# zhizdev/sparsefusion

Measured on AMD Instinct MI355X. Metric: novel views/sec, distillation steps (2 NGP renders fwd+bwd + VAE enc/dec + 51-eval PLMS + LPIPS), 256^2 / 32x32 latents, 2-view synthetic hydrant, higher is better.
Workload: dtype bf16 MFMA operands / f32 accumulate (UNet); f32 (NGP render)

## Files before the change

include/sparsefusion_hip.h:

```cpp
#ifndef SPARSEFUSION_HIP_H
#define SPARSEFUSION_HIP_H

#include <stdint.h>

#ifdef __cplusplus
extern "C" {
#endif

#define SF_OK 0
#define SF_ERR_INVALID 1
#define SF_ERR_LAUNCH 2

const char* sf_last_error(void);
int sf_abi_version(void);
int sf_operand_is_f16(void);


int sf_grid_encode_forward(const float* inputs, const float* embeddings,
                           const int32_t* offsets, float* outputs,
                           uint32_t B, uint32_t D, uint32_t C, uint32_t L,
                           float S, uint32_t H, float* dy_dx,
                           uint32_t gridtype, int align_corners,
                           const int32_t* h_offsets, void* stream);

// ... 188 lines not shown
  float* exp_avg;
  float* exp_avg_sq;
  uint64_t n;
  float step_size;
  float pad_;
} sf_adam_tensor;
typedef struct {
  sf_adam_tensor t[SF_ADAM_MAX_TENSORS];
  uint32_t chunk_start[SF_ADAM_MAX_TENSORS];
  uint32_t n_tensors;
  float beta1, beta2, eps;
  float bias_correction2_sqrt;
  float one_minus_beta1, one_minus_beta2;
} sf_adam_args;
int sf_adam_multi(const sf_adam_args* args, void* stream);

uint32_t sf_loss_partial_rows(void);
int sf_upsample2x_forward(const float* in, float* out, uint32_t planes, uint32_t h, uint32_t w, void* stream);
int sf_upsample2x_backward(const float* grad_out, float* grad_in, uint32_t planes, uint32_t h, uint32_t w, void* stream);
int sf_render_loss_forward(const float* img, const float* sil, const float* target_rgb, const float* target_mask, uint64_t n_img,
                           uint64_t n_sil, float scaling, float* partial, void* stream);
int sf_render_loss_backward(const float* img, const float* sil, const float* target_rgb, const float* target_mask, uint64_t n_img,
                            uint64_t n_sil, float scaling, float c_rgb, float c_sil, float c_opacity, float c_entropy,
                            const float* grad_loss, float* grad_img, float* grad_sil, void* stream);
int sf_fusion_loss_forward(const float* img, const float* pred, const float* view_weight, const float* sil, uint32_t views,
                           uint64_t per_view_img, uint64_t per_view_sil, float* partial, void* stream);
int sf_fusion_loss_backward(const float* img, const float* pred, const float* view_weight, const float* sil, uint32_t views,
                            uint64_t per_view_img, uint64_t per_view_sil, float c_l1, float c_opacity, float c_entropy,
                            const float* grad_loss, float* grad_img, float* grad_sil, void* stream);

int sf_plan_run(const sf_op* ops, uint32_t n_ops, void* stream);
uint64_t sf_conv_igemm_t_launches(void);
uint64_t sf_gca4_launches(int family);
int sf_plan_profile(const sf_op* ops, uint32_t n_ops, void* stream, float* h_ms);

uint64_t sf_conv_packed_elems(uint32_t Cout, uint32_t cin_pad, uint32_t kh, uint32_t kw);
int sf_conv_pack_weights(const float* h_w, uint32_t Cout, uint32_t Cin,
                         uint32_t cin_pad, uint32_t kh, uint32_t kw,
                         uint16_t* h_out);

int sf_plms_update(const float* x, const float* eps, const float* noise,
                   const float* h_coef6, uint64_t n, float* x_prev, float* x0,
                   void* stream);
int sf_plms_combine(const float* e0, const float* e1, const float* e2,
                    const float* e3, const float* h_c4, uint64_t n, float* out,
                    float* keep_e0, void* stream);
int sf_plms_step(const float* e0, const float* e1, const float* e2, const float* e3,
                 const float* h_c4, float* keep_e0, const float* x, const float* noise,
                 const float* h_coef6, uint64_t n, float* x_prev,
                 const float* row_src, float* row_dst, uint64_t row_n, void* stream);

#ifdef __cplusplus
}
#endif
#endif
```

sparsefusion_amd/_lib.py:

```python
import ctypes as C
import os

import torch

_HERE = os.path.dirname(os.path.abspath(__file__))
_DEFAULT_LIB = "libsparsefusion_hip_f16.so" if os.environ.get("SF_OPERAND", "bf16").lower() in ("f16", "fp16", "half") else "libsparsefusion_hip.so"
LIB_PATH = os.environ.get("SF_HIP_LIB") or os.path.join(_HERE, _DEFAULT_LIB)

_lib = None

c_f32p = C.c_void_p
c_i32p = C.c_void_p
u32 = C.c_uint32
u64 = C.c_uint64


class SfNgpField(C.Structure):
    _fields_ = [("embeddings", C.c_void_p), ("h_offsets", C.c_void_p), ("L", u32), ("S", C.c_float),
                ("H", u32), ("gridtype", u32),
                ("w0", C.c_void_p), ("b0", C.c_void_p), ("w1", C.c_void_p), ("b1", C.c_void_p),
                ("w2", C.c_void_p), ("b2", C.c_void_p), ("bound", C.c_float)]


class SfNgpFieldGrad(C.Structure):
# ... 56 lines not shown
                                          c_f32p, c_f32p, c_f32p, C.c_void_p]),
    "sf_ngp_density": (C.c_int, [C.POINTER(SfNgpField), c_f32p, u32, c_f32p, c_f32p, C.c_void_p]),
    "sf_ngp_density_lattice": (C.c_int, [C.POINTER(SfNgpField), c_f32p, c_f32p, c_f32p, u32, u32, u32, c_f32p, C.c_void_p]),
    "sf_ngp_point_attrs": (C.c_int, [C.POINTER(SfNgpField), c_f32p, u32, C.c_float, c_f32p, c_f32p, c_f32p, c_f32p, C.c_void_p]),
    "sf_ngp_texture_bake": (C.c_int, [C.POINTER(SfNgpField), c_f32p, u32, c_i32p, u32, u32, C.c_void_p, c_f32p, c_f32p, c_i32p,
                                      C.c_void_p]),
    "sf_gaussian3d_workspace_bytes": (u64, [u32, u32, u32]),
    "sf_gaussian3d": (C.c_int, [c_f32p, c_f32p, u32, u32, u32, C.c_float, C.c_float, C.c_void_p, C.c_void_p, u64, C.c_void_p]),
    "sf_mc_workspace_bytes": (u64, [u32, u32, u32]),
    "sf_mc_count": (C.c_int, [c_f32p, u32, u32, u32, C.c_float, C.c_void_p, u64, C.c_void_p, C.c_void_p]),
    "sf_mc_emit": (C.c_int, [c_f32p, u32, u32, u32, C.c_float, C.c_void_p, u64, c_f32p, c_i32p, C.c_void_p]),
    "sf_ngp_render_forward": (C.c_int, [C.POINTER(SfNgpField), c_f32p, c_f32p, c_f32p, u32, u32, C.c_float,
                                        c_f32p, c_f32p, c_f32p, u32, C.c_float, c_f32p, c_f32p, c_f32p, c_f32p,
                                        c_f32p, c_f32p, c_f32p, c_f32p, c_f32p, c_f32p, u64, C.c_void_p]),
    "sf_ngp_render_backward": (C.c_int, [C.POINTER(SfNgpField), C.POINTER(SfNgpFieldGrad), c_f32p, c_f32p,
                                         c_f32p, u32, u32, c_f32p, c_f32p, c_f32p, c_f32p, c_f32p,
                                         C.c_float, c_f32p, c_f32p, u32, c_f32p, c_f32p, u64, C.c_void_p]),
    "sf_ngp_render_workspace_bytes": (u64, [u32, u32]),
    "sf_ngp_render_forward_workspace_bytes": (u64, [u32, u32]),
    "sf_ngp_render_cache_bytes": (u64, [u32, u32]),
    "sf_ngp_render_shaded_forward": (C.c_int, [C.POINTER(SfNgpField), c_f32p, c_f32p, c_f32p, u32, u32, C.c_float, c_f32p, c_f32p,
                                               c_f32p, u32, C.c_float, c_f32p, C.c_float, C.c_float, c_f32p, c_f32p, c_f32p,
                                               c_f32p, c_f32p, c_f32p, c_f32p, c_f32p, c_f32p, c_f32p, c_f32p, c_f32p, c_f32p,
                                               c_f32p, u64, C.c_void_p]),
    "sf_ngp_render_shaded_workspace_bytes": (u64, [u32, u32]),
    "sf_ngp_render_occ_eval": (C.c_int, [C.POINTER(SfNgpField), c_f32p, c_f32p, c_f32p, c_f32p, C.c_void_p, C.c_float, u32, u32, u32,
                                         c_f32p, C.c_float, u32, c_f32p, c_f32p, c_f32p, C.c_void_p]),
    "sf_ngp_render_occ_eval_shaded": (C.c_int, [C.POINTER(SfNgpField), c_f32p, c_f32p, c_f32p, c_f32p, C.c_void_p, C.c_float, u32, u32,
                                                u32, c_f32p, C.c_float, u32, c_f32p, C.c_float, C.c_float, c_f32p, c_f32p, c_f32p,
                                                c_f32p, C.c_void_p, C.c_void_p]),
    "sf_plan_run": (C.c_int, [C.POINTER(SfOp), u32, C.c_void_p]),
    "sf_conv_igemm_t_launches": (u64, []),
    "sf_gca4_launches": (u64, [C.c_int]),
    "sf_plan_profile": (C.c_int, [C.POINTER(SfOp), u32, C.c_void_p, C.c_void_p]),
    "sf_conv_packed_elems": (u64, [u32, u32, u32, u32]),
    "sf_conv_pack_weights": (C.c_int, [C.c_void_p, u32, u32, u32, u32, u32, C.c_void_p]),
    "sf_plms_update": (C.c_int, [c_f32p, c_f32p, c_f32p, C.c_void_p, u64, c_f32p, c_f32p, C.c_void_p]),
    "sf_plms_combine": (C.c_int, [c_f32p, c_f32p, c_f32p, c_f32p, C.c_void_p, u64, c_f32p, c_f32p, C.c_void_p]),
    "sf_plms_step": (C.c_int, [c_f32p, c_f32p, c_f32p, c_f32p, C.c_void_p, c_f32p, c_f32p, c_f32p, C.c_void_p, u64, c_f32p, c_f32p, c_f32p, u64, C.c_void_p]),
}


_handles = {}


def _load(path):
    if path not in _handles:
        if not os.path.exists(path):
            raise RuntimeError(
                f"{path} is missing: build it with `python -m sparsefusion_amd.build` (`--f16` for the IEEE-half operand build; "
                "there is no CPU fallback for the sparsefusion_amd hot path)")
        handle = C.CDLL(path)
        for name, (res, args) in SIGNATURES.items():
            fn = getattr(handle, name)
            fn.restype = res
            fn.argtypes = args
        _handles[path] = handle
    return _handles[path]


def lib(operand=None):
    global _lib
    if operand is None:
        if _lib is None:
            _lib = _load(LIB_PATH)
        return _lib
# ... 30 lines not shown
```

sparsefusion_amd/csrc/unet_ops.hip:

```cpp

#include "sf_common.h"
#include "plan_ops.h"
#include "sf_dev.h"
#include "gemm_rows.h"
#include "conv_halo.h"
#include "conv_halo_small.h"
#include "conv_igemm.h"
#include "conv_igemm_t.h"
#include "attn_ln.h"
#include <math.h>

typedef __attribute__((ext_vector_type(8))) sf_opnd bf16x8;
typedef __attribute__((ext_vector_type(4))) sf_opnd bf16x4;
typedef __attribute__((ext_vector_type(4))) float f32x4;
typedef __attribute__((address_space(1))) float gfloat;

__device__ __forceinline__ void atomic_add_f32(float* p, float v) {
  (void)__builtin_amdgcn_global_atomic_fadd_f32((gfloat*)p, v);
}
__device__ __forceinline__ float silu_f(float v) { return v / (1.0f + __expf(-v)); }
__device__ __forceinline__ float sigmoid_f(float v) { return 1.0f / (1.0f + __expf(-v)); }
__device__ __forceinline__ float gelu_f(float v) { return 0.5f * v * (1.0f + erff(v * 0.70710678118654752f)); }

__device__ __forceinline__ float wave_sum(float v) {
#pragma unroll
  for (int o = 32; o > 0; o >>= 1) v += __shfl_xor(v, o, 64);
  return v;
}
__device__ __forceinline__ float wave_max(float v) {
#pragma unroll
  for (int o = 32; o > 0; o >>= 1) v = fmaxf(v, __shfl_xor(v, o, 64));
  return v;
}



__global__ __launch_bounds__(256) void k_splitk_reduce(const float* __restrict__ ws, const float* __restrict__ bias,
                                                       const float* __restrict__ resid, float* __restrict__ out, int M,
                                                       int Cout, int npad, int groups, int ldc, int co_off, int accum,
                                                       int relu, int nchw_hw) {
  const long total = (long)M * Cout;
  for (long i = blockIdx.x * 256L + threadIdx.x; i < total; i += (long)gridDim.x * 256) {
// ... 584 lines not shown
    SF_CHECK_LAUNCH("conv_lds");
    return conv_splitk_tail(op, a, M, st);
  }
  if ((op.flags & 512) && launch_conv_t(a, WM, WN, f32, blocks, st)) {
    SF_CHECK_LAUNCH("conv_igemm_t");
    return conv_splitk_tail(op, a, M, st);
  }
  switch (tile) {
    case 1 * 16 + 1: launch_conv<1, 1>(a, f32, blocks, st); break;
    case 1 * 16 + 2: launch_conv<1, 2>(a, f32, blocks, st); break;
    case 1 * 16 + 4: launch_conv<1, 4>(a, f32, blocks, st); break;
    case 2 * 16 + 1: launch_conv<2, 1>(a, f32, blocks, st); break;
    case 2 * 16 + 2: launch_conv<2, 2>(a, f32, blocks, st); break;
    case 2 * 16 + 4: launch_conv<2, 4>(a, f32, blocks, st); break;
    case 4 * 16 + 1: launch_conv<4, 1>(a, f32, blocks, st); break;
    case 4 * 16 + 2: launch_conv<4, 2>(a, f32, blocks, st); break;
    case 4 * 16 + 4: launch_conv<4, 4>(a, f32, blocks, st); break;
    default: SF_FAIL(SF_ERR_INVALID, "conv: unsupported wave tile %dx%d", WM, WN);
  }
  SF_CHECK_LAUNCH("conv_igemm");
  return conv_splitk_tail(op, a, M, st);
}

static int lazy_from_op(const sf_op& op, int ibase, int M, LazySrc& lz) {
  lz.mode = op.i[ibase]; lz.groups = op.i[ibase + 1]; lz.npad = op.i[ibase + 2]; lz.M = M;
  lz.a = (const float*)op.p[8]; lz.b = (const float*)op.p[9]; lz.r = (const float*)op.p[10];
  if (lz.mode < 0 || lz.mode > 2) SF_FAIL(SF_ERR_INVALID, "lazy source: unknown mode %d", lz.mode);
  if (lz.mode && !lz.a) SF_FAIL(SF_ERR_INVALID, "lazy source: missing operand");
  if (lz.mode == 1 && (lz.groups < 1 || lz.npad % 4)) SF_FAIL(SF_ERR_INVALID, "lazy source: bad split-K geometry");
  if (lz.mode == 2 && !lz.b) SF_FAIL(SF_ERR_INVALID, "lazy source: gate missing");
  return SF_OK;
}

static int run_gn(const sf_op& op, hipStream_t st) {
  const int B = op.i[0], HW = op.i[1], C1 = op.i[2], C2 = op.i[3];
  const int C = C1 + C2, G = op.i[8] > 0 ? op.i[8] : 8;
  if (C % (4 * G) || C1 % 4 || !op.p[7])
    SF_FAIL(SF_ERR_INVALID, "gn_act: unsupported shape HW=%d C=%d G=%d (or missing stats buffer)", HW, C, G);
  const int chunks = HW * (C / G) / 4;
  LazySrc lz;
  if (int rc = lazy_from_op(op, 5, B * HW, lz)) return rc;
  const int c4 = C / 4;
  if (!(op.flags & (2 | 4)) && (B * G >= 256 || (B * G >= 64 && (long)B * HW * C <= (1L << 19)) || (op.flags & 8)) && chunks <= 1024 * 16) {
    float* s1 = (float*)op.p[0];
    const float *s2 = (const float*)op.p[1], *ga = (const float*)op.p[2], *be = (const float*)op.p[3], *ssp = (const float*)op.p[4];
    sf_opnd *o = (sf_opnd*)op.p[5], *rw = (sf_opnd*)op.p[6];
#define SF_GN_ONE(NT, NCH) k_gn_one<NT, NCH><<<B * G, NT, 0, st>>>(s1, s2, ga, be, ssp, o, rw, HW, C1, C2, op.i[4], op.f[0], op.f[1], op.flags & 1, lz, G)
    if (chunks <= 256 * 2) SF_GN_ONE(256, 2);
    else if (chunks <= 256 * 4) SF_GN_ONE(256, 4);
    else if (chunks <= 256 * 8) SF_GN_ONE(256, 8);
    else if (chunks <= 256 * 16) SF_GN_ONE(256, 16);
    else if (chunks <= 1024 * 8) SF_GN_ONE(1024, 8);
    else SF_GN_ONE(1024, 16);
#undef SF_GN_ONE
    SF_CHECK_LAUNCH("gn_one");
    return SF_OK;
  }
  if (op.flags & 2) {
    if (op.p[1] || lz.mode) SF_FAIL(SF_ERR_INVALID, "gn_act: ready-made statistics need a plain single source");
  } else if (!op.p[1] && !lz.mode && C / G <= 16 && c4 <= 256 && 256 % c4 == 0) {
    const int ppi = 256 / c4;
    int slabs = HW / (ppi * 16);
    slabs = slabs < 1 ? 1 : (slabs > 1024 ? 1024 : slabs);
    k_gn_stats_px<<<B * slabs, 256, 0, st>>>((const float*)op.p[0], (double*)op.p[7], HW, C, G, slabs);
  } else {
    const int per_block = lz.mode == 1 ? 256 : GN_CHUNKS_PER_BLOCK;
    int slices = (chunks + per_block - 1) / per_block;
    const int want = 128 / (B * G), max_slices = (chunks + 255) / 256;
    if (slices < want) slices = want < max_slices ? want : max_slices;
    if (slices < 1) slices = 1;
    k_gn_stats<<<B * G * slices, 256, 0, st>>>((float*)op.p[0], (const float*)op.p[1], (double*)op.p[7], HW, C1, C2, slices,
                                               op.f[1], lz, G);
  }
  SF_CHECK_LAUNCH("gn_stats");
  const long total = (long)B * HW * (C / 4);
  k_gn_apply<<<sf_grid_cap(sf_div_up(total, 256)), 256, 0, st>>>(
      (const float*)op.p[0], (const float*)op.p[1], (const float*)op.p[2], (const float*)op.p[3], (const float*)op.p[4],
      (const double*)op.p[7], (sf_opnd*)op.p[5], (sf_opnd*)op.p[6], B, HW, C1, C2, op.i[4], op.f[0], op.f[1], op.flags & 1, G);
  SF_CHECK_LAUNCH("gn_apply");
  return SF_OK;
}

static int run_ln(const sf_op& op, hipStream_t st) {
  const int R = op.i[0], C = op.i[1];
  if (C % 64 || C > 2048) SF_FAIL(SF_ERR_INVALID, "layernorm: C must be a multiple of 64 and <= 2048");
  if (C == 256 && R >= 1024) {
    k_layernorm_w256<<<sf_div_up(R, 4), 256, 0, st>>>((const float*)op.p[0], (const float*)op.p[1], (const float*)op.p[2], op.p[3],
                                                      (const float*)op.p[4], R, op.f[0], op.flags & 1, (op.flags & 2) ? 1 : 0, (sf_opnd*)op.p[5]);
    SF_CHECK_LAUNCH("layernorm_w256");
    return SF_OK;
  }
  if (op.p[5]) SF_FAIL(SF_ERR_INVALID, "layernorm: the operand-type twin output exists for >= 1024 rows of 256 channels only");
// ... 134 lines not shown
    if (ev && hipEventRecord(ev[k], st) != hipSuccess) SF_FAIL(SF_ERR_LAUNCH, "plan: hipEventRecord failed");
    switch (op.type) {
      case SF_OP_CONV: rc = run_conv(op, st); break;
      case SF_OP_GN_ACT: rc = run_gn(op, st); break;
      case SF_OP_LN: rc = run_ln(op, st); break;
      case SF_OP_GEMV: rc = run_gemv(op, st); break;
      case SF_OP_ATTN: rc = run_attn(op, st); break;
      case SF_OP_GCA_POOL: rc = run_gca_pool(op, st); break;
      case SF_OP_ELTWISE: rc = run_eltwise(op, st); break;
      case SF_OP_MEMSET:
        if (hipMemsetAsync(op.p[0], 0, (size_t)(uint32_t)op.i[0] * 4, st) != hipSuccess) SF_FAIL(SF_ERR_LAUNCH, "memset failed");
        break;
      case SF_OP_SPLITK_REDUCE: {
        const int M = op.i[0], Cout = op.i[1];
        if (!op.p[0] || !op.p[3] || op.i[3] < 1) SF_FAIL(SF_ERR_INVALID, "splitk_reduce: bad operands");
        k_splitk_reduce<<<sf_grid_cap(sf_div_up((long)M * Cout, 256)), 256, 0, st>>>(
            (const float*)op.p[0], (const float*)op.p[1], (const float*)op.p[2], (float*)op.p[3], M, Cout, op.i[2], op.i[3], Cout, 0, 0, 0, 0);
        if (hipGetLastError() != hipSuccess) SF_FAIL(SF_ERR_LAUNCH, "splitk_reduce launch failed");
        break;
      }
      case SF_OP_TIME_EMB:
        k_time_emb<<<sf_div_up(op.i[0] * op.i[1], 64), 64, 0, st>>>((const float*)op.p[0], (const float*)op.p[1], (float*)op.p[3],
                                                                  op.i[0], op.i[1]);
        if (hipGetLastError() != hipSuccess) SF_FAIL(SF_ERR_LAUNCH, "time_emb launch failed");
        break;
      case SF_OP_POOL:
      case SF_OP_LPIPS: rc = sf_plan_extra_op(&op, st); break;
      case SF_OP_EFT: rc = sf_plan_eft_op(&op, st); break;
      case SF_OP_INITX: rc = sf_plan_initx_op(&op, st); break;
      case SF_OP_GN_FINALIZE: {
        const int G = op.i[2];
        if (!op.p[0] || !op.p[1] || op.i[0] < 1 || op.i[1] < 1 || G < 1 || G > 256 || 256 % G)
          SF_FAIL(SF_ERR_INVALID, "gn_finalize: bad operands");
        k_gn_finalize<<<op.i[0] * G, 256, 0, st>>>((const double*)op.p[0], (double*)op.p[1], op.i[1], G);
        SF_CHECK_LAUNCH("gn_finalize");
        rc = SF_OK;
        break;
      }
      case SF_OP_FCONV:
        if (op.flags & 16) {
          if (k + 1 >= n_ops) SF_FAIL(SF_ERR_INVALID, "plan: a paired fconv needs a successor");
          rc = sf_plan_fused_pair(&op, &ops[k + 1], st);
          if (!rc) {
            ++k;
            if (ev && hipEventRecord(ev[k], st) != hipSuccess) SF_FAIL(SF_ERR_LAUNCH, "plan: hipEventRecord failed");
          }
          break;
        }
        rc = sf_plan_fused_op(&op, st);
        break;
      case SF_OP_SLOTS:
      case SF_OP_GCA: rc = sf_plan_fused_op(&op, st); break;
      default: SF_FAIL(SF_ERR_INVALID, "plan: unknown op type %d at %u", op.type, k);
    }
    if (rc) {
      char tmp[400];
      snprintf(tmp, sizeof(tmp), "%s", sf_err_buf);
      snprintf(sf_err_buf, sizeof(sf_err_buf), "plan op %u (type %d): %s", k, op.type, tmp);
      return rc;
    }
  }
  if (ev && hipEventRecord(ev[n_ops], st_main) != hipSuccess) SF_FAIL(SF_ERR_LAUNCH, "plan: hipEventRecord failed");
  return SF_OK;
}

extern "C" int sf_plan_run(const sf_op* ops, uint32_t n_ops, void* stream) {
  return plan_run_impl(ops, n_ops, (hipStream_t)stream, nullptr);
}

extern "C" int sf_plan_profile(const sf_op* ops, uint32_t n_ops, void* stream, float* h_ms) {
  hipStream_t st = (hipStream_t)stream;
  hipEvent_t* ev = new hipEvent_t[n_ops + 1];
  uint32_t made = 0;
  int rc = SF_OK;
  for (; made <= n_ops; ++made)
    if (hipEventCreate(&ev[made]) != hipSuccess) { rc = SF_ERR_LAUNCH; break; }
  if (rc == SF_OK) rc = plan_run_impl(ops, n_ops, st, ev);
  else snprintf(sf_err_buf, sizeof(sf_err_buf), "plan_profile: hipEventCreate failed");
  if (rc == SF_OK && hipEventSynchronize(ev[n_ops]) != hipSuccess) rc = SF_ERR_LAUNCH;
  for (uint32_t k = 0; k < n_ops && rc == SF_OK; ++k)
    if (hipEventElapsedTime(&h_ms[k], ev[k], ev[k + 1]) != hipSuccess) rc = SF_ERR_LAUNCH;
  for (uint32_t k = 0; k < made; ++k) (void)hipEventDestroy(ev[k]);
  delete[] ev;
  return rc;
}

#if SF_OPERAND_F16
static inline uint16_t f32_to_bf16_rne(float f) {
  const _Float16 h = (_Float16)f;
  uint16_t u;
  memcpy(&u, &h, 2);
  return u;
}
#else
static inline uint16_t f32_to_bf16_rne(float f) {
  uint32_t u;
  memcpy(&u, &f, 4);
  if ((u & 0x7fffffffu) > 0x7f800000u) return (uint16_t)((u >> 16) | 0x40);
  u += 0x7fffu + ((u >> 16) & 1u);
  return (uint16_t)(u >> 16);
}
#endif
// ... 118 lines not shown
```

sparsefusion_amd/lpips.py:

```python
import math

import os
import torch
import torch.nn as nn

from . import _lib
from .plan import OP_ELTWISE, OP_MEMSET, Plan, PlanOwner, _T
from .unet import _register

OP_POOL, OP_LPIPS = 11, 12
SHIFT = (-.030, -.088, -.188)
SCALE = (.458, .448, .450)
VGG_CONVS = [(1, 0, 3, 64), (1, 2, 64, 64), (2, 5, 64, 128), (2, 7, 128, 128), (3, 10, 128, 256), (3, 12, 256, 256),
             (3, 14, 256, 256), (4, 17, 256, 512), (4, 19, 512, 512), (4, 21, 512, 512), (5, 24, 512, 512),
             (5, 26, 512, 512), (5, 28, 512, 512)]
CHNS = (64, 128, 256, 512, 512)


def lpips_param_spec():
    spec = []
    for sl, idx, cin, cout in VGG_CONVS:
        spec += [(f"net.slice{sl}.{idx}.weight", (cout, cin, 3, 3)), (f"net.slice{sl}.{idx}.bias", (cout,))]
    for k, c in enumerate(CHNS):
        spec.append((f"lin{k}.model.1.weight", (1, c, 1, 1)))
# ... 60 lines not shown
        g = grads[id(f.taps[-1][0])]
        H = f.taps[-1][1]
        for ci in reversed(range(len(VGG_CONVS))):
            sl, idx, cin, cout = VGG_CONVS[ci]
            y = f.conv_out[ci]
            gz = self.bf16(V * H * H, cout, H * H)
            self.op(OP_ELTWISE, 7, p=(g.ptr, y.ptr, 0, gz.ptr), i=(V * H * H * cout,))
            cpad = 32 if cin == 3 else cin
            gx = self.f32(V * H * H, cpad, H * H)
            name = f"net.slice{sl}.{idx}"
            self.conv(gz, False, H, H, name + ".weight.T", None, gx, cpad, 0, cpad, 3, 1, 1)
            g = gx
            if ci in f.pool_in:
                src, Hs = f.pool_in[ci]
                gt = grads[id(src)]
                gp = self.f32(V * Hs * Hs, src.C, Hs * Hs)
                self.op(OP_POOL, 1, p=(g.ptr, src.ptr, 0, gp.ptr), i=(V, Hs, Hs, src.C))
                self.op(OP_ELTWISE, 4, p=(gp.ptr, 0, 0, gt.ptr), i=(V * Hs * Hs * src.C,))
                g, H = gt, Hs
        self.out = self.f32(V, 3 * R * R)
        self.op(OP_ELTWISE, 9, p=(g.ptr, self.wptr("__scaling__"), 0, self.out.ptr), i=(V, R * R, 32))
        self.op_array = (_lib.SfOp * len(self.ops))(*self.ops)
        if self.misc.buf is not None:
            self.out_view, self.gscale_view = self.tview(self.out), self.tview(self.gscale)
        return self


class _LpipsFn(torch.autograd.Function):
    @staticmethod
    def forward(ctx, mod, pred, target):
        V = pred.shape[0]
        fwd, bwd = mod._plans_for(V, pred.shape[-1], pred.device)
        fwd.x_view.copy_(torch.cat([pred, target], 0).reshape(2 * V, -1))
        _lib.check(mod.clib.sf_plan_run(fwd.op_array, len(fwd.ops), _lib.stream_ptr()), "lpips forward plan", mod.clib)
        ctx.mod, ctx.bwd, ctx.shape = mod, bwd, pred.shape
        ctx.serial = mod._serial = mod._serial + 1
        return fwd.dist_view.clone().view(V, 1, 1, 1)

    @staticmethod
    def backward(ctx, g):
        if ctx.serial != ctx.mod._serial:
            raise RuntimeError("PerceptualLoss: backward after another forward -- the feature maps live in one static arena")
        bwd = ctx.bwd
        mod = ctx.mod
        sc = mod.grad_scale
        g = g.reshape(-1, 1).float()
        if sc == 1.0:
            bwd.gscale_view.copy_(g)
        else:
            gmax = g.abs().max().clamp_min(1e-30)
            bwd.gscale_view.copy_(g * (sc / gmax))
        _lib.check(mod.clib.sf_plan_run(bwd.op_array, len(bwd.ops), _lib.stream_ptr()), "lpips backward plan", mod.clib)
        out = bwd.out_view.clone() if sc == 1.0 else bwd.out_view * (gmax / sc)
        return None, out.view(ctx.shape), None


class LPIPS(PlanOwner, nn.Module):

    def __init__(self, net='vgg', verbose=False, **unsupported):
        super().__init__()
        if net not in ('vgg', 'vgg16'):
            raise NotImplementedError("only net='vgg' is used by the reference (distillation.py:161)")
        g = torch.Generator().manual_seed(0)
        for name, shape in lpips_param_spec():
            if name.startswith("lin"):
                t = torch.rand(shape, generator=g) / shape[1] * 4
            elif name.endswith("bias"):
                t = torch.zeros(shape)
            else:
                t = torch.randn(shape, generator=g) * math.sqrt(2.0 / (shape[1] * 9))
            _register(self, name, nn.Parameter(t, requires_grad=False))
        self.lds_conv_min_blocks = 96
        self.conv_twin = True
        self._pack_cache, self._plans, self._serial = None, {}, 0
        self.operand, self.grad_scale = None, 1.0
        self._weights_loaded = False

    def invalidate(self):
        self._pack_cache, self._plans = None, {}

    def set_operand(self, operand, grad_scale=None):
        if operand not in (None, "bf16", "f16"):
            raise ValueError("operand must be None, 'bf16' or 'f16'")
        self.operand = operand
        self.grad_scale = float(grad_scale if grad_scale is not None else (4096.0 if operand == "f16" else 1.0))
# ... 103 lines not shown
```

sparsefusion_amd/plan.py:

```python
import torch

from . import _lib

OP_CONV, OP_GN_ACT, OP_LN, OP_GEMV, OP_ATTN, OP_GCA_POOL, OP_ELTWISE, OP_MEMSET, OP_TIME_EMB, OP_SPLITK_REDUCE = range(1, 11)
OP_FCONV, OP_SLOTS, OP_GCA, OP_INITX, OP_GN_FINALIZE = 14, 15, 16, 17, 18
FNORM_NONE, FNORM_GN_SELF, FNORM_GN_SLOTS, FNORM_LN, FNORM_ATTN = range(5)
LDS_MAX = 163840
SKIP_SCALE = 2 ** -0.5


class _Arena:

    def __init__(self, nbytes=None, device=None):
        self.off = 0
        self.buf = torch.empty(nbytes, dtype=torch.uint8, device=device) if nbytes else None

    def alloc(self, nbytes):
        nbytes = (nbytes + 255) // 256 * 256
        off = self.off
        self.off += nbytes
        return (self.buf.data_ptr() + off) if self.buf is not None else (1 << 20) + off


class _T:
    __slots__ = ("ptr", "rows", "C", "HW", "lazy", "slots", "writer", "twin")

    def __init__(self, ptr, rows, C, HW=None):
        self.ptr, self.rows, self.C, self.HW = ptr, rows, C, HW
        self.lazy = None
        self.slots = None
        self.twin = None
        self.writer = None


class PlanOwner:
# ... 16 lines not shown
        if ov and (m_frags, n_frags, KS, bool(pixshuf)) in ov:
            return ov[(m_frags, n_frags, KS, bool(pixshuf))]
        best = None
        mfma = m_frags * n_frags * KS
        w_bytes = n_frags * KS * 1024
        for WM in (1, 2, 4):
            if m_frags % WM or (m_frags <= 4 and WM != m_frags and m_frags in (1, 2, 4)):
                continue
            for WN in (1, 2, 4):
                if n_frags % WN:
                    continue
                tiles = (m_frags // WM) * (n_frags // WN)
                for groups in ((1,) if pixshuf else (1, 2, 4, 8, 16, 32)):
                    if groups > 1 and KS // (4 * groups) < 2:
                        continue
                    waves = tiles * groups * 4
                    util = min(1.0, waves / self.conv_waves_target)
                    t_hbm = w_bytes / 4.0e12 / util
                    t_l2 = mfma * 1024 * (1.0 / WN + 1.0 / WM) / 12.0e12 / util
                    t_mfma = mfma * 20 / (1024 * 2.1e9) / util
                    t_part = (2.0 * groups * m_frags * n_frags * 1024 / 3.0e12 + 2.0e-6) if groups > 1 else 0.0
                    cost = max(t_hbm, t_l2, t_mfma) + t_part + 1e-9 * WM * WN
                    if best is None or cost < best[0]:
                        best = (cost, WM, WN, groups)
        return best[1], best[2], best[3]


class Plan:

    def __init__(self, unet, B, device, sizing=None):
        self.u, self.B, self.dev = unet, B, device
        self.ops = []
        self.graph = None
        if sizing is None:
            self.zero, self.misc = _Arena(), _Arena()
        else:
            self.zero, self.misc = _Arena(sizing[0], device), _Arena(sizing[1], device)
        self.w = unet._packed(device)
        self.written = set()
        self.ws_need = [0, 0]
        self.ws_ptrs = [self.misc.alloc(sizing[2]) if sizing is not None else 0,
                        self.misc.alloc(sizing[3]) if sizing is not None and len(sizing) > 3 and sizing[3] else 0]
        self.ws_owners = [None, None]

    @property
    def ws_bytes(self):
        return self.ws_need[0]

    @property
    def ws2_bytes(self):
        return self.ws_need[1]

    @property
    def ws_owner(self):
        return next((o for o in self.ws_owners if o is not None and o.lazy is not None), None)

    def acquire_ws(self, nbytes, avoid=()):
        for i in sorted(range(2), key=lambda j: (self.ws_owners[j] is not None and self.ws_owners[j].lazy is not None, j)):
            o = self.ws_owners[i]
            if o is not None and o.lazy is not None:
                if any(o is t for t in avoid):
                    continue
                self.need(o)
            self.ws_need[i] = max(self.ws_need[i], nbytes)
            self.ws_owners[i] = None
            return i
        raise AssertionError("no split-K workspace available")

    def f32(self, rows, C, HW=None):
        return _T(self.misc.alloc(rows * C * 4), rows, C, HW)

    def bf16(self, rows, C, HW=None):
        return _T(self.misc.alloc(rows * C * 2), rows, C, HW)

    def op(self, type_, flags=0, p=(), i=(), f=()):
        o = _lib.SfOp()
# ... 156 lines not shown
```

sparsefusion_amd/unet.py:

```python
import math
import os

import numpy as np
import torch
import torch.nn as nn

from . import _lib
from .plan import (FNORM_ATTN, FNORM_GN_SELF, FNORM_GN_SLOTS, FNORM_LN, FNORM_NONE, LDS_MAX, OP_ATTN, OP_CONV, OP_ELTWISE, OP_FCONV, OP_GCA,
                   OP_GCA_POOL, OP_GEMV, OP_GN_ACT, OP_GN_FINALIZE, OP_INITX, OP_LN, OP_MEMSET, OP_SLOTS, OP_SPLITK_REDUCE, OP_TIME_EMB,
                   SKIP_SCALE, Plan, PlanOwner, _T)

PAIR_TILES = {(1, 1, 1), (1, 1, 2), (1, 2, 2), (2, 2, 2), (4, 2, 2)}
PIPE_TILES = {(1, 1, 4), (1, 2, 4), (1, 1, 6), (1, 2, 6), (2, 1, 6), (2, 2, 6), (2, 1, 8), (2, 2, 8), (2, 1, 12), (2, 2, 12), (4, 1, 16), (4, 2, 16)}
CONV3S_VARIANTS = {(5, 256, 5, 2, 2), (5, 256, 3, 2, 2), (4, 256, 4, 1, 1), (4, 256, 2, 1, 1), (4, 512, 4, 1, 2), (4, 512, 2, 1, 2),
                   (3, 512, 3, 1, 1), (3, 1024, 3, 1, 1), (5, 256, 5, 4, 2), (5, 256, 3, 4, 2),
                   (4, 256, 2, 2, 1), (4, 256, 2, 2, 2), (4, 512, 2, 2, 2), (3, 512, 3, 2, 1), (3, 1024, 3, 2, 1), (3, 1024, 3, 2, 2)}
CONV3S_RC_VARIANTS = {(5, 256, 256, 256, 3, 2, 2), (4, 512, 256, 512, 2, 1, 2), (3, 1024, 512, 1024, 3, 1, 1)}
IGEMM_T_VARIANTS = ((5, 256, 256, 4, 2, 1, 0, 2, 2, 4, 1, 0), (4, 256, 512, 4, 2, 1, 0, 1, 2, 8, 1, 0), (3, 512, 1024, 4, 2, 1, 0, 1, 1, 4, 1, 0),
                    (2, 1024, 4096, 1, 1, 0, 0, 1, 1, 1, 1, 1), (3, 1024, 2048, 1, 1, 0, 0, 1, 1, 1, 1, 1), (4, 512, 1024, 1, 1, 0, 0, 1, 2, 1, 1, 1),
                    (5, 256, 4, 3, 1, 1, 0, 1, 1, 4, 1, 0))
ATTN_LDS_BYTES = 8 * 16 * 36 * 4 + 2 * 8 * 4 * 68 * 4
TILE_PICKS = {(4, 32, 128, False): (1, 2, 8),
              (4, 128, 32, True): (1, 1, 1),
              (16, 64, 16, True): (1, 2, 1),
# ... 1063 lines not shown
    @staticmethod
    def _run_plan(plan, body_only=False):
        if body_only:
            _lib.check(plan.u.clib.sf_plan_run(plan.body_array, plan.n_body_ops, _lib.stream_ptr()), "unet plan", plan.u.clib)
        else:
            _lib.check(plan.u.clib.sf_plan_run(plan.op_array, len(plan.ops), _lib.stream_ptr()), "unet plan", plan.u.clib)

    def _time_plan(self, T, device):
        key = ("time", T, str(device))
        if key not in self._plans:
            old = [k for k in self._plans if k[0] == "time"]
            for k in old[:max(0, len(old) + 1 - self.MAX_TIME_PLANS)]:
                del self._plans[k]
            sizing = _TimePlan(self, T, device).build()
            self._plans[key] = _TimePlan(self, T, device, (sizing.zero.off, sizing.misc.off + 512, 0, 0)).build()
        else:
            self._plans[key] = self._plans.pop(key)
        return self._plans[key]

    @torch.no_grad()
    def time_table(self, log_snrs, key=None):
        _lib.require_cuda(log_snrs)
        ck = None
        if key is not None:
            ck = (key, str(log_snrs.device), self.operand)
            hit = self.__dict__.get("_table_cache", {}).get(ck)
            if hit is not None:
                cache = self.__dict__["_table_cache"]
                cache[ck] = cache.pop(ck)
                return hit
        T = log_snrs.numel()
        plan = self._time_plan(T, log_snrs.device)
        plan.t_view.copy_(log_snrs.reshape(T, 1))
        _lib.check(self.clib.sf_plan_run(plan.op_array, len(plan.ops), _lib.stream_ptr()), "unet time plan", self.clib)
        table = plan.table_view.clone()
        if ck is not None:
            cache = self.__dict__.setdefault("_table_cache", {})
            while len(cache) >= 2:
                cache.pop(next(iter(cache)))
            cache[ck] = table
        return table

    @torch.no_grad()
    def begin_sampling(self, cond_images, log_snrs, table_key=None):
        _lib.require_cuda(cond_images)
        B = cond_images.shape[0]
        if cond_images.shape[-1] != self.image_size:
            cond_images = torch.nn.functional.interpolate(cond_images, self.image_size, mode='nearest')
        plan = self._plan(B, cond_images.device)
        plan.generation += 1
        plan.cond_view.copy_(cond_images.reshape(B, -1))
        plan.x_view.zero_()
        _lib.check(self.clib.sf_plan_run(plan.init_array, plan.n_init_run, _lib.stream_ptr()), "unet init conv", self.clib)
        plan.base_view.copy_(plan.x0_view)
        return {"plan": plan, "table": self.time_table(log_snrs, key=table_key), "B": B, "generation": plan.generation}

    @torch.no_grad()
    def eval_prepared(self, ctx, x, row, row_ready=False):
        plan, B = ctx["plan"], ctx["B"]
        if ctx.get("generation") != plan.generation:
            raise RuntimeError("Unet.eval_prepared: this sampling context is stale -- a later forward() / begin_sampling() with the same "
                               "batch size, or invalidate() / .to(), took over the plan that held its latents and time rows; "
                               "call begin_sampling() again")
        if x.data_ptr() != plan.x_view.data_ptr():
            plan.x_view.copy_(x.reshape(B, -1))
        if not row_ready:
            plan.tb_view.copy_(ctx["table"][row].expand(B, -1))
# ... 28 lines not shown
```

sparsefusion_amd/vae.py:

```python
import math

import numpy as np
import os

import torch
import torch.nn as nn

from . import _lib
from .plan import OP_ELTWISE, OP_MEMSET, Plan, PlanOwner, _T
from .unet import _register

SD_VAE_DDCONFIG = dict(double_z=True, z_channels=4, resolution=256, in_channels=3, out_ch=3, ch=128, ch_mult=(1, 2, 4, 4),
                       num_res_blocks=2, attn_resolutions=(), dropout=0.0)


def _resnet_spec(out, p, cin, cout):
    out += [(f"{p}.norm1.weight", (cin,)), (f"{p}.norm1.bias", (cin,)), (f"{p}.conv1.weight", (cout, cin, 3, 3)),
            (f"{p}.conv1.bias", (cout,)), (f"{p}.norm2.weight", (cout,)), (f"{p}.norm2.bias", (cout,)),
            (f"{p}.conv2.weight", (cout, cout, 3, 3)), (f"{p}.conv2.bias", (cout,))]
    if cin != cout:
        out += [(f"{p}.nin_shortcut.weight", (cout, cin, 1, 1)), (f"{p}.nin_shortcut.bias", (cout,))]


def _attn_spec(out, p, c):
# ... 269 lines not shown
        return r

    def _packed(self, device):
        if self._pack_cache is not None and self._pack_cache[0] == str(device):
            return self._pack_cache[1]
        lib = _lib.lib()
        packed = {}
        for name, w in self.named_parameters():
            wc = w.detach().float().cpu().contiguous()
            if wc.dim() == 4:
                co, ci, kh, kw = wc.shape
                cpad = (ci + 31) // 32 * 32
                buf = torch.empty(lib.sf_conv_packed_elems(co, cpad, kh, kw), dtype=torch.int16)
                _lib.check(lib.sf_conv_pack_weights(wc.data_ptr(), co, ci, cpad, kh, kw, buf.data_ptr()), "pack " + name)
                packed[name] = buf.to(device)
            else:
                packed[name] = wc.reshape(-1).to(device)
        self._pack_cache = (str(device), packed)
        return packed

    def _plan(self, kind, B, device):
        key = (kind, B, str(device))
        if key not in self._plans:
            sizing = _VaePlan(self, kind, B, device).build()
            self._plans[key] = _VaePlan(self, kind, B, device,
                                        (sizing.zero.off, sizing.misc.off + sizing.ws_bytes + 256, sizing.ws_bytes)).build()
        return self._plans[key]

    def _run(self, kind, x):
        _lib.require_cuda(x)
        B = x.shape[0]
        plan = self._plan(kind, B, x.device)
        plan.x_view.copy_(x.reshape(B, -1))
        _lib.check(_lib.lib().sf_plan_run(plan.op_array, len(plan.ops), _lib.stream_ptr()), f"vae {kind} plan")
        return plan.out_view.clone().view(B, *plan.out_shape)

    @torch.no_grad()
    def encode(self, x):
        assert x.shape[1:] == (self.in_channels, self.resolution, self.resolution), x.shape
        return DiagonalGaussianDistribution(self._run("enc", x.float()))

    @torch.no_grad()
    def decode(self, z):
        f = 2 ** (len(self.ch_mult) - 1)
        assert z.shape[1:] == (self.embed_dim, self.resolution // f, self.resolution // f), z.shape
        return self._run("dec", z.float())

    def forward(self, input, sample_posterior=True):
        posterior = self.encode(input)
        z = posterior.sample() if sample_posterior else posterior.mode()
        return self.decode(z), posterior
```

Measured before the change: 18.13.

## Add fused GroupNorm-ready kernel folding finalize, and optional HIP graph replay for plans

Adds a k_gn_ready kernel that applies GroupNorm with ready statistics, optional scale-shift and SiLU, and writes bf16 output. When a gn_finalize op is followed by a compatible gn_act, the kernel also folds the finalize reduction of per-tile partial sums into the same launch, removing one kernel and a round trip through the stats buffer. Separately, plan execution for the VAE, LPIPS and UNet time-embedding plans can be captured into a HIP graph and replayed to cut per-op launch overhead. Graph replay only turns on when SF_PLAN_GRAPH=1, so by default only the fused GN path is active. The folded reduction uses shared-memory trees with double-precision slots and is limited in tile count.

```diff
diff --git a/include/sparsefusion_hip.h b/include/sparsefusion_hip.h
--- a/include/sparsefusion_hip.h
+++ b/include/sparsefusion_hip.h
@@ -244,6 +244,10 @@
 int sf_plan_run(const sf_op* ops, uint32_t n_ops, void* stream);
 uint64_t sf_conv_igemm_t_launches(void);
 uint64_t sf_gca4_launches(int family);
+uint64_t sf_gn_ready_launches(int form);
+int sf_plan_graph_create(const sf_op* ops, uint32_t n_ops, void* stream, void** handle);
+int sf_plan_graph_launch(void* handle, void* stream);
+int sf_plan_graph_destroy(void* handle);
 int sf_plan_profile(const sf_op* ops, uint32_t n_ops, void* stream, float* h_ms);
 
 uint64_t sf_conv_packed_elems(uint32_t Cout, uint32_t cin_pad, uint32_t kh, uint32_t kw);
diff --git a/sparsefusion_amd/_lib.py b/sparsefusion_amd/_lib.py
--- a/sparsefusion_amd/_lib.py
+++ b/sparsefusion_amd/_lib.py
@@ -112,6 +112,10 @@
     "sf_plan_run": (C.c_int, [C.POINTER(SfOp), u32, C.c_void_p]),
     "sf_conv_igemm_t_launches": (u64, []),
     "sf_gca4_launches": (u64, [C.c_int]),
+    "sf_gn_ready_launches": (u64, [C.c_int]),
+    "sf_plan_graph_create": (C.c_int, [C.POINTER(SfOp), u32, C.c_void_p, C.POINTER(C.c_void_p)]),
+    "sf_plan_graph_launch": (C.c_int, [C.c_void_p, C.c_void_p]),
+    "sf_plan_graph_destroy": (C.c_int, [C.c_void_p]),
     "sf_plan_profile": (C.c_int, [C.POINTER(SfOp), u32, C.c_void_p, C.c_void_p]),
     "sf_conv_packed_elems": (u64, [u32, u32, u32, u32]),
     "sf_conv_pack_weights": (C.c_int, [C.c_void_p, u32, u32, u32, u32, u32, C.c_void_p]),
diff --git a/sparsefusion_amd/csrc/gn_ready.h b/sparsefusion_amd/csrc/gn_ready.h
--- /dev/null
+++ b/sparsefusion_amd/csrc/gn_ready.h
@@ -0,0 +1,77 @@
+#pragma once
+#include "sf_dev.h"
+
+#define GN_READY_FOLD_SLOTS 1024
+
+SF_KERNEL(256) void k_gn_ready(const float* __restrict__ x, const float* __restrict__ gamma, const float* __restrict__ beta,
+                               const float* __restrict__ ss, double* __restrict__ stats, const double* __restrict__ part,
+                               sf_opnd* __restrict__ out, sf_opnd* __restrict__ raw, int HW, int C, int G, int ss_stride, float eps,
+                               int no_silu, int tiles, int lgP, int ppb, int bpi) {
+  SF_SHARED double red[2][GN_READY_FOLD_SLOTS];
+  SF_SHARED float mr[2][256];
+  const int tid = threadIdx.x;
+  const int b = blockIdx.x / bpi, blk = blockIdx.x - b * bpi;
+  const int Cg = C / G, c4 = C >> 2;
+  if (part) {
+    const int P = 1 << lgP;
+    for (int j = tid; j < tiles * G; j += 256) {
+      const int t = j / G, g = j - t * G;
+      const double* p = part + ((long)b * tiles * G + j) * 2;
+      red[0][(g << lgP) + t] = 0.0 + p[0];
+      red[1][(g << lgP) + t] = 0.0 + p[1];
+    }
+    for (int j = tid; j < (P - tiles) * G; j += 256) {
+      const int t = j / G, g = j - t * G;
+      red[0][(g << lgP) + tiles + t] = 0.0;
+      red[1][(g << lgP) + tiles + t] = 0.0;
+    }
+    sf_sync();
+    for (int lw = lgP - 1; lw >= 0; --lw) {
+      for (int j = tid; j < (G << lw); j += 256) {
+        const int g = j >> lw, t = j - (g << lw);
+        const int k = (g << lgP) + t;
+        red[0][k] += red[0][k + (1 << lw)];
+        red[1][k] += red[1][k + (1 << lw)];
+      }
+      sf_sync();
+    }
+  }
+  if (tid < G) {
+    const int g = tid;
+    const double sum = part ? red[0][g << lgP] : stats[(b * G + g) * 2];
+    const double sq = part ? red[1][g << lgP] : stats[(b * G + g) * 2 + 1];
+    const double inv_n = 1.0 / ((double)HW * Cg);
+    const double m = sum * inv_n;
+    const double var = sq * inv_n - m * m;
+    const float mean = (float)m, rstd = sf_rsqrt((float)(var > 0.0 ? var : 0.0) + eps);
+    mr[0][g] = mean; mr[1][g] = rstd;
+    if (part && blk == 0) { stats[(b * G + g) * 2] = sum; stats[(b * G + g) * 2 + 1] = sq; }
+  }
+  sf_sync();
+  const int pofs = tid / c4, chunk = tid - pofs * c4, ppi = 256 / c4;
+  const int c = chunk * 4, g = c / Cg;
+  const float mean = mr[0][g], rstd = mr[1][g];
+  const f32x4 ga = *reinterpret_cast<const f32x4*>(gamma + c), be = *reinterpret_cast<const f32x4*>(beta + c);
+  f32x4 sc = {0.f, 0.f, 0.f, 0.f}, sh = {0.f, 0.f, 0.f, 0.f};
+  if (ss) {
+    sc = *reinterpret_cast<const f32x4*>(ss + (long)b * ss_stride + c);
+    sh = *reinterpret_cast<const f32x4*>(ss + (long)b * ss_stride + C + c);
+  }
+  const int p0 = blk * ppb, p1 = p0 + ppb < HW ? p0 + ppb : HW;
+#pragma unroll 4
+  for (int p = p0 + pofs; p < p1; p += ppi) {
+    const int at = (b * HW + p) * C + c;
+    const f32x4 v = *reinterpret_cast<const f32x4*>(x + at);
+    bf16x4 o, r;
+#pragma unroll
+    for (int j = 0; j < 4; ++j) {
+      float y = (v[j] - mean) * rstd * ga[j] + be[j];
+      if (ss) y = y * (sc[j] + 1.0f) + sh[j];
+      if (!no_silu) y = sf_silu(y);
+      o[j] = (sf_opnd)y;
+      r[j] = (sf_opnd)v[j];
+    }
+    *reinterpret_cast<bf16x4*>(out + at) = o;
+    if (raw) *reinterpret_cast<bf16x4*>(raw + at) = r;
+  }
+}
diff --git a/sparsefusion_amd/csrc/unet_ops.hip b/sparsefusion_amd/csrc/unet_ops.hip
--- a/sparsefusion_amd/csrc/unet_ops.hip
+++ b/sparsefusion_amd/csrc/unet_ops.hip
@@ -8,6 +8,7 @@
 #include "conv_igemm.h"
 #include "conv_igemm_t.h"
 #include "attn_ln.h"
+#include "gn_ready.h"
 #include <math.h>
 
 typedef __attribute__((ext_vector_type(8))) sf_opnd bf16x8;
@@ -658,6 +659,50 @@
   return SF_OK;
 }
 
+static uint64_t g_gn_ready_launches[2];
+extern "C" uint64_t sf_gn_ready_launches(int form) { return (form == 0 || form == 1) ? g_gn_ready_launches[form] : 0; }
+
+#define GN_READY_FOLD_MAX_TILES 16
+
+static bool gn_ready_ok(const sf_op& op) {
+  const int B = op.i[0], HW = op.i[1], C = op.i[2], G = op.i[8] > 0 ? op.i[8] : 8;
+  if ((op.flags & 4) || !(op.flags & 2) || op.p[1] || op.i[3] || op.i[5]) return false;
+  if (B < 1 || HW < 1 || C < 4 || C % (4 * G) || G > 256) return false;
+  const int c4 = C / 4;
+  if (c4 > 256 || 256 % c4 || (long)B * HW * C >= (1L << 31)) return false;
+  if (((uintptr_t)op.p[0] | (uintptr_t)op.p[2] | (uintptr_t)op.p[3] | (uintptr_t)op.p[4]) & 15) return false;
+  if (op.p[4] && op.i[4] % 4) return false;
+  return op.p[0] && op.p[2] && op.p[3] && op.p[5] && op.p[7];
+}
+
+static int gn_ready_lgP(int tiles) {
+  int lg = 0;
+  while ((1 << lg) < tiles) ++lg;
+  return lg;
+}
+
+static bool gn_ready_folds(const sf_op& fin, const sf_op& act) {
+  if (act.type != SF_OP_GN_ACT || !gn_ready_ok(act)) return false;
+  const int tiles = fin.i[1], G = fin.i[2];
+  if (!fin.p[0] || act.p[7] != fin.p[1] || act.i[0] != fin.i[0] || (act.i[8] > 0 ? act.i[8] : 8) != G || tiles < 1) return false;
+  if ((act.i[1] + 127) / 128 != tiles || tiles > 256 || (G << gn_ready_lgP(tiles)) > GN_READY_FOLD_SLOTS) return false;
+  return tiles <= GN_READY_FOLD_MAX_TILES || (act.flags & 8);
+}
+
+static int run_gn_ready(const sf_op& op, hipStream_t st, const double* part, int tiles) {
+  const int B = op.i[0], HW = op.i[1], C = op.i[2], G = op.i[8] > 0 ? op.i[8] : 8;
+  const int ppi = 256 / (C / 4);
+  int it = 4;
+  while (it > 1 && (long)B * sf_div_up(HW, ppi * it) < (it == 4 ? 1024 : 512)) it >>= 1;
+  const int ppb = ppi * it, bpi = (int)sf_div_up(HW, ppb);
+  k_gn_ready<<<B * bpi, 256, 0, st>>>((const float*)op.p[0], (const float*)op.p[2], (const float*)op.p[3], (const float*)op.p[4],
+                                      (double*)op.p[7], part, (sf_opnd*)op.p[5], (sf_opnd*)op.p[6], HW, C, G, op.i[4], op.f[0],
+                                      op.flags & 1, part ? tiles : 0, part ? gn_ready_lgP(tiles) : 0, ppb, bpi);
+  SF_CHECK_LAUNCH("gn_ready");
+  ++g_gn_ready_launches[part ? 1 : 0];
+  return SF_OK;
+}
+
 static int run_gn(const sf_op& op, hipStream_t st) {
   const int B = op.i[0], HW = op.i[1], C1 = op.i[2], C2 = op.i[3];
   const int C = C1 + C2, G = op.i[8] > 0 ? op.i[8] : 8;
@@ -684,6 +729,7 @@
   }
   if (op.flags & 2) {
     if (op.p[1] || lz.mode) SF_FAIL(SF_ERR_INVALID, "gn_act: ready-made statistics need a plain single source");
+    if (gn_ready_ok(op)) return run_gn_ready(op, st, nullptr, 0);
   } else if (!op.p[1] && !lz.mode && C / G <= 16 && c4 <= 256 && 256 % c4 == 0) {
     const int ppi = 256 / c4;
     int slabs = HW / (ppi * 16);
@@ -884,6 +930,14 @@
         const int G = op.i[2];
         if (!op.p[0] || !op.p[1] || op.i[0] < 1 || op.i[1] < 1 || G < 1 || G > 256 || 256 % G)
           SF_FAIL(SF_ERR_INVALID, "gn_finalize: bad operands");
+        if (k + 1 < n_ops && gn_ready_folds(op, ops[k + 1])) {
+          rc = run_gn_ready(ops[k + 1], st, (const double*)op.p[0], op.i[1]);
+          if (!rc) {
+            ++k;
+            if (ev && hipEventRecord(ev[k], st) != hipSuccess) SF_FAIL(SF_ERR_LAUNCH, "plan: hipEventRecord failed");
+          }
+          break;
+        }
         k_gn_finalize<<<op.i[0] * G, 256, 0, st>>>((const double*)op.p[0], (double*)op.p[1], op.i[1], G);
         SF_CHECK_LAUNCH("gn_finalize");
         rc = SF_OK;
@@ -920,6 +974,74 @@
   return plan_run_impl(ops, n_ops, (hipStream_t)stream, nullptr);
 }
 
+struct sf_plan_graph { hipGraphExec_t exec; };
+
+extern "C" int sf_plan_graph_create(const sf_op* ops, uint32_t n_ops, void* stream, void** handle) {
+  hipStream_t st = (hipStream_t)stream;
+  if (!handle) SF_FAIL(SF_ERR_INVALID, "plan_graph_create: null handle pointer");
+  *handle = nullptr;
+  hipStreamCaptureStatus cs = hipStreamCaptureStatusNone;
+  if (hipStreamIsCapturing(st, &cs) != hipSuccess || cs != hipStreamCaptureStatusNone) {
+    (void)hipGetLastError();
+    snprintf(sf_err_buf, sizeof(sf_err_buf), "plan_graph_create: the stream is being captured already; plain launches");
+    return SF_OK;
+  }
+  if (int rc = plan_run_impl(ops, n_ops, st, nullptr)) return rc;
+  if (hipStreamSynchronize(st) != hipSuccess) SF_FAIL(SF_ERR_LAUNCH, "plan_graph_create: the warm-up run failed");
+  hipStream_t cap = st, own = nullptr;
+  if (!st || st == hipStreamLegacy) {
+    if (hipStreamCreateWithFlags(&own, hipStreamNonBlocking) != hipSuccess) {
+      (void)hipGetLastError();
+      snprintf(sf_err_buf, sizeof(sf_err_buf), "plan_graph_create: no capture stream; plain launches");
+      return SF_OK;
+    }
+    cap = own;
+  }
+  hipError_t e = hipStreamBeginCapture(cap, hipStreamCaptureModeThreadLocal);
+  int rc = SF_OK;
+  hipGraph_t g = nullptr;
+  hipGraphExec_t ge = nullptr;
+  size_t roots = 0;
+  const char* why = "hipStreamBeginCapture";
+  if (e == hipSuccess) {
+    rc = plan_run_impl(ops, n_ops, cap, nullptr);
+    e = hipStreamEndCapture(cap, &g);
+    why = rc ? "an op under capture" : "hipStreamEndCapture";
+    if (rc == SF_OK && e == hipSuccess && g) {
+      why = "not a linear chain";
+      if (hipGraphGetRootNodes(g, nullptr, &roots) == hipSuccess && roots == 1) {
+        why = "hipGraphInstantiate";
+        e = hipGraphInstantiate(&ge, g, nullptr, nullptr, 0);
+      }
+    }
+  }
+  if (g) (void)hipGraphDestroy(g);
+  if (own) (void)hipStreamDestroy(own);
+  if (!ge) {
+    (void)hipGetLastError();
+    snprintf(sf_err_buf, sizeof(sf_err_buf), "plan_graph_create: %s failed (%s); plain launches", why, hipGetErrorString(e));
+    return SF_OK;
+  }
+  *handle = new sf_plan_graph{ge};
+  return SF_OK;
+}
+
+extern "C" int sf_plan_graph_launch(void* handle, void* stream) {
+  if (!handle) SF_FAIL(SF_ERR_INVALID, "plan_graph_launch: null handle");
+  if (hipGraphLaunch(((sf_plan_graph*)handle)->exec, (hipStream_t)stream) != hipSuccess) SF_FAIL(SF_ERR_LAUNCH, "plan_graph_launch: hipGraphLaunch failed");
+  return SF_OK;
+}
+
+extern "C" int sf_plan_graph_destroy(void* handle) {
+  if (!handle) return SF_OK;
+  sf_plan_graph* h = (sf_plan_graph*)handle;
+  (void)hipDeviceSynchronize();
+  const hipError_t e = hipGraphExecDestroy(h->exec);
+  delete h;
+  if (e != hipSuccess) SF_FAIL(SF_ERR_LAUNCH, "plan_graph_destroy: hipGraphExecDestroy failed");
+  return SF_OK;
+}
+
 extern "C" int sf_plan_profile(const sf_op* ops, uint32_t n_ops, void* stream, float* h_ms) {
   hipStream_t st = (hipStream_t)stream;
   hipEvent_t* ev = new hipEvent_t[n_ops + 1];
diff --git a/sparsefusion_amd/lpips.py b/sparsefusion_amd/lpips.py
--- a/sparsefusion_amd/lpips.py
+++ b/sparsefusion_amd/lpips.py
@@ -116,7 +116,7 @@
         V = pred.shape[0]
         fwd, bwd = mod._plans_for(V, pred.shape[-1], pred.device)
         fwd.x_view.copy_(torch.cat([pred, target], 0).reshape(2 * V, -1))
-        _lib.check(mod.clib.sf_plan_run(fwd.op_array, len(fwd.ops), _lib.stream_ptr()), "lpips forward plan", mod.clib)
+        fwd.run("lpips forward plan", mod.clib)
         ctx.mod, ctx.bwd, ctx.shape = mod, bwd, pred.shape
         ctx.serial = mod._serial = mod._serial + 1
         return fwd.dist_view.clone().view(V, 1, 1, 1)
@@ -134,7 +134,7 @@
         else:
             gmax = g.abs().max().clamp_min(1e-30)
             bwd.gscale_view.copy_(g * (sc / gmax))
-        _lib.check(mod.clib.sf_plan_run(bwd.op_array, len(bwd.ops), _lib.stream_ptr()), "lpips backward plan", mod.clib)
+        bwd.run("lpips backward plan", mod.clib)
         out = bwd.out_view.clone() if sc == 1.0 else bwd.out_view * (gmax / sc)
         return None, out.view(ctx.shape), None
 
diff --git a/sparsefusion_amd/plan.py b/sparsefusion_amd/plan.py
--- a/sparsefusion_amd/plan.py
+++ b/sparsefusion_amd/plan.py
@@ -1,6 +1,21 @@
+import ctypes
+import os
+import weakref
+
 import torch
 
 from . import _lib
+
+PLAN_GRAPH_COUNTS = {"created": 0, "replayed": 0, "plain": 0}
+
+
+def plan_graph_enabled():
+    return os.environ.get("SF_PLAN_GRAPH", "0") == "1"
+
+
+def _destroy_plan_graph(clib, handle):
+    clib.sf_plan_graph_destroy(ctypes.c_void_p(handle))
+
 
 OP_CONV, OP_GN_ACT, OP_LN, OP_GEMV, OP_ATTN, OP_GCA_POOL, OP_ELTWISE, OP_MEMSET, OP_TIME_EMB, OP_SPLITK_REDUCE = range(1, 11)
 OP_FCONV, OP_SLOTS, OP_GCA, OP_INITX, OP_GN_FINALIZE = 14, 15, 16, 17, 18
@@ -83,6 +98,7 @@
         self.u, self.B, self.dev = unet, B, device
         self.ops = []
         self.graph = None
+        self.replay = None
         if sizing is None:
             self.zero, self.misc = _Arena(), _Arena()
         else:
@@ -93,6 +109,30 @@
         self.ws_ptrs = [self.misc.alloc(sizing[2]) if sizing is not None else 0,
                         self.misc.alloc(sizing[3]) if sizing is not None and len(sizing) > 3 and sizing[3] else 0]
         self.ws_owners = [None, None]
+
+    def run(self, what, clib=None):
+        clib = clib or _lib.lib()
+        if plan_graph_enabled() and self.replay is not False:
+            if torch.cuda.is_current_stream_capturing():
+                if self.replay is None:
+                    self.replay = False
+            else:
+                if self.replay is None:
+                    h = ctypes.c_void_p()
+                    _lib.check(clib.sf_plan_graph_create(self.op_array, len(self.ops), _lib.stream_ptr(), ctypes.byref(h)), what, clib)
+                    self.replay = h.value or False
+                    if not self.replay:
+                        import warnings
+                        warnings.warn(f"sparsefusion_amd: {what}: {clib.sf_last_error().decode('utf-8', 'replace')}")
+                    else:
+                        PLAN_GRAPH_COUNTS["created"] += 1
+                        weakref.finalize(self, _destroy_plan_graph, clib, h.value).atexit = False
+                if self.replay:
+                    _lib.check(clib.sf_plan_graph_launch(ctypes.c_void_p(self.replay), _lib.stream_ptr()), what, clib)
+                    PLAN_GRAPH_COUNTS["replayed"] += 1
+                    return
+        _lib.check(clib.sf_plan_run(self.op_array, len(self.ops), _lib.stream_ptr()), what, clib)
+        PLAN_GRAPH_COUNTS["plain"] += 1
 
     @property
     def ws_bytes(self):
diff --git a/sparsefusion_amd/unet.py b/sparsefusion_amd/unet.py
--- a/sparsefusion_amd/unet.py
+++ b/sparsefusion_amd/unet.py
@@ -1119,7 +1119,7 @@
         T = log_snrs.numel()
         plan = self._time_plan(T, log_snrs.device)
         plan.t_view.copy_(log_snrs.reshape(T, 1))
-        _lib.check(self.clib.sf_plan_run(plan.op_array, len(plan.ops), _lib.stream_ptr()), "unet time plan", self.clib)
+        plan.run("unet time plan", self.clib)
         table = plan.table_view.clone()
         if ck is not None:
             cache = self.__dict__.setdefault("_table_cache", {})
diff --git a/sparsefusion_amd/vae.py b/sparsefusion_amd/vae.py
--- a/sparsefusion_amd/vae.py
+++ b/sparsefusion_amd/vae.py
@@ -325,7 +325,7 @@
         B = x.shape[0]
         plan = self._plan(kind, B, x.device)
         plan.x_view.copy_(x.reshape(B, -1))
-        _lib.check(_lib.lib().sf_plan_run(plan.op_array, len(plan.ops), _lib.stream_ptr()), f"vae {kind} plan")
+        plan.run(f"vae {kind} plan")
         return plan.out_view.clone().view(B, *plan.out_shape)
 
     @torch.no_grad()
```

Result: no change. 18.10 (-0.2%).
